# hritikbharucha/Custom_Porechop_ABI

Measured on AMD Instinct MI355X. Metric: reads/sec trimmed (100k ONT reads x 50 adapter pairs), higher is better.
Workload: dtype int32

## Files before the change

### custom_porechop_abi_amd/csrc/pcabi_dp.h

```cpp
#pragma once

#ifndef PCABI_ROW_FENCE
#define PCABI_ROW_FENCE 1
#endif
#ifndef PCABI_TAB_PD
#define PCABI_TAB_PD 0
#endif
#ifndef PCABI_TAB_PD_LONG
#define PCABI_TAB_PD_LONG 1
#endif

#include <stdint.h>
#include <algorithm>

#ifdef __HIPCC__
#define PCABI_HD __host__ __device__ __forceinline__
#else
#define PCABI_HD inline
#endif

namespace pcabi {

constexpr int NEG = -(1 << 28);

// ... 423 lines not shown
            best.b.bj = j;
            const int vt = LAST ? vt_up : 0, vp = LAST ? vp_up : 0;
            if (AFFINE) {
                if (lv == ls)      { best.c = lvc; best.n = lvn; best.b.ltype = LT_V; best.b.trail = vt; best.b.precd = vp; }
                else if (lh == ls) { best.c = lhc; best.n = lhn; best.b.ltype = LT_H; best.b.trail = ht; best.b.precd = hp; }
                else               { best.c = lsc; best.n = lsn; best.b.ltype = LT_D; best.b.trail = 0; best.b.precd = 0; }
            } else {
                best.c = lsc; best.n = lsn; best.b.ltype = lt_type;
                best.b.trail = (lt_type == LT_V) ? vt : (lt_type == LT_H ? ht : 0);
                best.b.precd = (lt_type == LT_V) ? vp : (lt_type == LT_H ? hp : 0);
            }
        }
        if (AFFINE || lt_type == LT_H) { ht_last = ht; hp_last = hp; }
        else { ht_last = 0; hp_last = 0; }
        slt_last = lt_type;
    }
};

template <int R, bool AFFINE, typename ReadFn, typename AdpFn, typename BndFn>
PCABI_HD Result align_lane_striped(const ReadFn &rd0, int n, AdpFn &adp, int L, int rt, const Scoring sc, BndFn &bnd,
                                   int own_lo = 1, int own_hi = -1) {
    const bool fin_read = own_hi < 0;
    const int hi = fin_read ? n + 1 : own_hi;
    const int pad = rt - L, k0 = pad / R, nst = rt / R;
    StripeDP<R, AFFINE> st;
    st.best.b.score = 0;
    st.best.b.bi = L;
    st.best.b.bj = 0;
    st.best.b.attr = 0;
    st.best.b.ltype = LT_NONE;
    st.best.b.trail = 0;
    st.best.b.precd = 0;
    st.best.c = -L;
    st.best.n = 0;
    st.bc = st.best;
    st.bc.b.score = SCORE_FLOOR;
    st.cslt = LT_NONE;
    st.cvt = 0;
    st.cvp = 0;
#pragma unroll 1
    for (int k = k0; k < nst; ++k) {
        adp.load(k);
        const bool first = k == k0, fin = k == nst - 1;
        const int off = first ? pad - k0 * R : 0;
        const int ib = k * R - pad;
        st.init_stripe(ib, off);
        ReadFn rd = rd0;
        BndCell up, nx, bot;
        auto row0 = [](int j, BndCell &u) { u.s = 0; u.v = NEG; u.sc = j; u.vc = 0; u.sn = 0; u.vn = 0; };
        if (first) row0(1, up);
        else bnd.load(1, up);
        int r = rd(1);
#pragma unroll 1
        for (int j = 1; j < n; ++j) {
            const int rn = rd(j + 1);
            if (first) row0(j + 1, nx);
            else bnd.load(j + 1, nx);
            st.template column<false>(r, j, up, adp, off, ib, L, fin, j >= own_lo && j < hi, sc, bot);
            if (!fin) bnd.store(j, bot);
            up = nx;
            r = rn;
        }
        if (fin_read) st.template column<true>(r, n, up, adp, off, ib, L, fin, n >= own_lo && n < hi, sc, bot);
        else st.template column<false>(r, n, up, adp, off, ib, L, fin, n >= own_lo && n < hi, sc, bot);
        if (!fin) bnd.store(n, bot);
    }
    return finish_path(st.best.b, st.best.c, (int)(st.best.n & 0xFFFFu), (int)(st.best.n >> 16), L,
                       fin_read ? n : n + 1);
}

}

namespace pcabi {

constexpr uint32_t INC_PAD = 1u << ATTR_CSH;

PCABI_HD int32_t vreg(int32_t x) {
#if defined(__HIP_DEVICE_COMPILE__)
    asm volatile("" : "+v"(x));
#endif
    return x;
}

PCABI_HD int max3i(int a, int b, int c) {
    const int ab = a > b ? a : b;
    return ab > c ? ab : c;
}
constexpr int PAD_CODE = 5;

template <int RPL, bool AFFINE>
struct LaneDP {
    int S[RPL + 1], H[RPL + 1];
    uint32_t SA[RPL + 1], HA[RPL + 1];
    int bscore, bi, bj, blt, btrail, bprec;
    uint32_t battr;
    int slt_last, ht_last, hp_last;
    int mis[4];
    uint32_t ids[4];

    template <typename AdpFn, bool LAST>
    PCABI_HD void column(const int r, const int j, const AdpFn &adp, const int L, const int off,
                         const Scoring &sc) {
        int sup = 0, vup = NEG;
        uint32_t saup = attr_start(j), vaup = 0;
        int slt_up = LT_NONE, vt_up = 0, vp_up = 0;
        int lv = 0, lh = 0, ls = 0, lslt = LT_D;
        bool lhext = false;
        uint32_t lva = 0, lha = 0, lsa = 0;
        bool match = (r == adp(1));
        int diag = 0 + (match ? sc.ma : mis[1]);
        uint32_t da = attr_start(j - 1) + ids[1] + (uint32_t)match;
#pragma unroll
        for (int s = 1; s <= RPL; ++s) {
            int diag_nx = 0;
            uint32_t da_nx = 0;
            if (s < RPL) {
                const bool mt = (r == adp(s + 1));
                const int mi_n = (s + 1 <= 3) ? mis[s + 1] : sc.mi;
                const uint32_t id_n = (s + 1 <= 3) ? ids[s + 1] : INC_D;
                diag_nx = S[s] + (mt ? sc.ma : mi_n);
                da_nx = SA[s] + id_n + (uint32_t)mt;
            }
            int hn, vn, sn;
            uint32_t han, van;
            bool hext, vext, fromv;
            if (AFFINE) {
                const int hx = H[s] + sc.ge, ho = S[s] + sc.go;
                hext = !(hx < ho);
                hn = hext ? hx : ho;
                han = hext ? HA[s] : SA[s];
                const int vx = vup + sc.ge, vo = sup + sc.go;
                vext = !(vx < vo);
                vn = vext ? vx : vo;
                van = vext ? vaup : saup;
            } else {
                hext = vext = false;
                vn = sup + sc.ge;
                hn = S[s] + sc.ge;
                van = saup;
                han = SA[s];
            }
            sn = max3i(diag, vn, hn);
            const bool isd = (diag == sn);
            fromv = (vn == sn);
            const uint32_t san = isd ? da : (fromv ? van : han);
            if (LAST && s < RPL) {
                const int slt = isd ? LT_D : (fromv ? LT_V : LT_H);
                const bool cont = AFFINE ? (vext || slt_up == LT_V) : (slt_up == LT_V);
                const int vt = cont ? vt_up + 1 : 1;
                const int vp = cont ? vp_up : (slt_up == LT_D ? 1 : 0);
                if (sn > bscore) {
                    bscore = sn;
                    bi = s - off;
                    bj = j;
                    if (AFFINE) {
                        const bool isv = (vn == sn), ish = !isv && (hn == sn);
                        battr = isv ? van : (ish ? han : san);
                        blt = isv ? LT_V : (ish ? LT_H : LT_D);
                        btrail = isv ? vt : 0;
                        bprec = isv ? vp : 0;
                    } else {
                        battr = san;
                        blt = slt;
                        btrail = (slt == LT_V) ? vt : 0;
                        bprec = (slt == LT_V) ? vp : 0;
                    }
// ... 632 lines not shown
    PCABI_HD void init(int L, const Scoring &sc, int P_, int B, int j0 = 0) {
        using pk::addw;
        const int off = RPL - L;
        P = P_;
        jj = j0;
        k_e = Y::sc(-sc.ge);
        k_eR = Y::sc(-sc.ge * RPL);
        k_rb = Y::sc(sc.ge * P);
        f0 = Y::sc(-B);
        kgo0 = Y::sc(sc.go - sc.ge) + ((P - 1) << Y::TB_SH);
        ftop = Y::sc(-sc.ge * j0 - B);
        kgo = kgo0 - j0 * Y::TAG1;
        int32_t fs = addw(ftop, kgo);
#pragma unroll
        for (int s = 1; s <= RPL; ++s) {
            fs = addw(fs, k_e);
            st.G[s] = addw(Y::start(off - s), fs);
            st.HK[s] = addw(fs, Y::sc(-1) + Y::TAG1);
        }
        st.bkey = Y::start(-L);
        st.bj = 0;
    }

    PCABI_HD void step() {
        ++jj;
        kgo -= Y::TAG1;
        ftop = pk::addw(ftop, k_e);
    }

    PCABI_HD void advance() {
        using pk::addw;
        step();
        if (jj == P) {
            const int32_t rb = addw(k_rb, P << Y::TB_SH);
#pragma unroll
            for (int s = 1; s <= RPL; ++s) {
                st.G[s] = addw(st.G[s], rb);
                st.HK[s] = addw(st.HK[s], rb);
            }
            jj = 0;
            kgo += P << Y::TB_SH;
            ftop = addw(ftop, k_rb);
        }
    }

    template <typename TabRow>
    PCABI_HD void column(const TabRow &tab, const int j, const int off) {
        using pk::addw;
        const int32_t kg = vreg(kgo);
        const int32_t top = addw(ftop, kgo);
        int32_t gup = addw(Y::start(j + off), top);
        int32_t vup = Y::SENT;
        int32_t diag = addw(addw(Y::start(j - 1 + off), top), Y::TAG1 - k_e);
        constexpr int NQ = RPL / 4;
        int32_t t[RPL + 2];
        if (PD > 0) {
#pragma unroll
            for (int q = 0; q <= PD && q < NQ; ++q) tab.quad(q, t + 4 * q + 1);
        }
        diag += (PD > 0 ? t[1] : tab(1));
        int32_t lv = 0, ls = 0;
#pragma unroll
        for (int s = 1; s <= RPL; ++s) {
            if (PD > 0 && (s & 3) == 1) {
                const int q = (s - 1) / 4 + PD + 1;
                if (q < NQ) tab.quad(q, t + 4 * q + 1);
            }
            int32_t diag_nx = 0;
            if (s < RPL) diag_nx = st.G[s] + (PD > 0 ? t[s + 1] : tab(s + 1));
            const int32_t hn = std::max(st.HK[s], st.G[s]);
            const int32_t vo = gup + Y::kv(s);
            const int32_t vn = std::max(vup, vo);
            const int32_t sn = max3i(diag, vn, hn);
            if (s == RPL) { lv = vn; ls = sn; }
            st.G[s] = (sn & ~Y::TAGM) + kg;
            st.HK[s] = hn;
            gup = st.G[s];
            vup = vn;
            diag = diag_nx;
#if defined(__HIP_DEVICE_COMPILE__)
            if (PCABI_ROW_FENCE > 0 && (s % (PCABI_ROW_FENCE > 0 ? PCABI_ROW_FENCE : 1)) == 0) __builtin_amdgcn_sched_barrier(0);
#endif
        }
        const int32_t corr = addw(std::max(lv, ls & ~Y::TAGM), pk::negw(addw(ftop, k_eR)));
        const bool upd = Y::score(corr) > Y::score(st.bkey);
        st.bkey = upd ? corr : st.bkey;
        st.bj = upd ? j : st.bj;
    }

    template <typename TabRow>
    PCABI_HD Result last_column(const TabRow &tab, const int n, const int L) {
        using pk::addw;
        using pk::negw;
        const int off = RPL - L;
        const int32_t ft = addw(f0, (int32_t)((uint32_t)jj * (uint32_t)k_e));
        const int32_t kgj = kgo0 - jj * Y::TAG1;
        const int32_t kg = vreg(kgj);
        const int32_t top = addw(ft, kgj);
        int32_t gup = addw(Y::start(n + off), top);
        int32_t vup = Y::SENT;
        int32_t diag = addw(addw(Y::start(n - 1 + off), top), Y::TAG1 - k_e);
        constexpr int NQ = RPL / 4;
        int32_t t[RPL + 2];
        if (PD > 0) {
#pragma unroll
            for (int q = 0; q <= PD && q < NQ; ++q) tab.quad(q, t + 4 * q + 1);
        }
        diag += (PD > 0 ? t[1] : tab(1));
        int32_t bkey = st.bkey;
        int brow = 0;
        int32_t un = negw(ft);
#pragma unroll
        for (int s = 1; s <= RPL; ++s) {
            if (PD > 0 && (s & 3) == 1) {
                const int q = (s - 1) / 4 + PD + 1;
                if (q < NQ) tab.quad(q, t + 4 * q + 1);
            }
            int32_t diag_nx = 0;
            if (s < RPL) diag_nx = st.G[s] + (PD > 0 ? t[s + 1] : tab(s + 1));
            const int32_t hn = std::max(st.HK[s], st.G[s]);
            const int32_t vo = gup + Y::kv(s);
            const int32_t vn = std::max(vup, vo);
            const int32_t sn = max3i(diag, vn, hn);
            const int32_t s0 = sn & ~Y::TAGM;
            un = addw(un, negw(k_e));
            const int32_t corr = addw(std::max(hn, s0), un);
            const bool upd = Y::score(corr) > Y::score(bkey);
            bkey = upd ? corr : bkey;
            brow = upd ? s : brow;
            gup = s0 + kg;
            vup = vn;
            diag = diag_nx;
#if defined(__HIP_DEVICE_COMPILE__)
            if (PCABI_ROW_FENCE > 0 && (s % (PCABI_ROW_FENCE > 0 ? PCABI_ROW_FENCE : 1)) == 0) __builtin_amdgcn_sched_barrier(0);
#endif
        }
        const bool last = brow != 0, tagged = Y::tb(bkey) != 0;
        Best b;
        b.score = Y::score(bkey);
        b.bi = last ? brow - off : L;
        b.bj = last ? n : st.bj;
        b.attr = Y::to_std(Y::attr(bkey), b.bj);
        b.ltype = last ? (tagged ? LT_H : LT_D) : (st.bj == 0 ? LT_NONE : (tagged ? LT_V : LT_D));
        b.trail = 0;
        b.precd = 0;
        return finish(b, L, n);
    }
};

template <int RPL, int PD = PCABI_TAB_PD, typename ReadFn, typename TabFn>
PCABI_HD Result align_lane_shift(ReadFn &rd, int n, const TabFn &tabfn, int L, const Scoring sc, int P, int B) {
    LaneShift<RPL, PD> ls;
    const int off = RPL - L;
    ls.init(L, sc, P, B);
    int r = rd(1);
#pragma unroll 1
    for (int j = 1; j < n; ++j) {
        const int rn = rd(j + 1);
        ls.advance();
        ls.template column<decltype(tabfn(r))>(tabfn(r), j, off);
        r = rn;
    }
    ls.advance();
    return ls.template last_column<decltype(tabfn(r))>(tabfn(r), n, L);
}

template <int RPL, int PD = PCABI_TAB_PD, typename TileFn, typename TabFn>
PCABI_HD Result align_lane_shift4(const TileFn &tr, int n, const TabFn &tabfn, int L, const Scoring sc, int P, int B) {
    LaneShift<RPL, PD> ls;
    const int off = RPL - L;
    ls.init(L, sc, P, B, -1);
    const int np = (n - 1) / 4;
    uint32_t cur = tr(0), nx = tr(1);
    int j = 1;
#pragma unroll 1
    for (int q = 0; q < np; ++q, j += 4) {
        const uint32_t w = cur;
        cur = nx;
        nx = tr(q + 2);
        ls.advance();
        ls.template column<decltype(tabfn(0))>(tabfn((int)(w & 0xFFu)), j, off);
        ls.step();
        ls.template column<decltype(tabfn(0))>(tabfn((int)((w >> 8) & 0xFFu)), j + 1, off);
        ls.step();
        ls.template column<decltype(tabfn(0))>(tabfn((int)((w >> 16) & 0xFFu)), j + 2, off);
        ls.step();
        ls.template column<decltype(tabfn(0))>(tabfn((int)(w >> 24)), j + 3, off);
    }
#pragma unroll 1
    for (; j < n; ++j) {
        ls.advance();
        ls.template column<decltype(tabfn(0))>(tabfn((int)((cur >> (8 * ((j - 1) & 3))) & 0xFFu)), j, off);
    }
    ls.advance();
    return ls.template last_column<decltype(tabfn(0))>(tabfn((int)((cur >> (8 * ((n - 1) & 3))) & 0xFFu)), n, L);
}

namespace pk {
template <int RPL, typename AdpFn>
PCABI_HD int32_t sub_key_pshift(int s, int c, const AdpFn &adp, int off, const Scoring &sc) {
    using Y = Lay<RPL>;
    const int d = -sc.go - sc.ge;
    if (s <= off) return Y::TB3 + Y::sc(d);
    return (c == adp(s)) ? (Y::sc(sc.ma + d) + Y::TB3 + Y::INC_M) : (Y::sc(sc.mi + d) + Y::TB3 + Y::INC_D);
}
constexpr int32_t PSENT = (int32_t)0x80000000;
}

template <int RPL, int PD = PCABI_TAB_PD>
struct LanePShift {
    using Y = pk::Lay<RPL>;
    LanePacked<RPL, true, Y, PD> st;
    int32_t kgo;
    int32_t ftop;
    int32_t f0;
    int32_t k_e;
    int32_t k_eR;
    int32_t k_rb;
    int jj, P;

    PCABI_HD void init(int L, const Scoring &sc, int P_, int B) {
        using pk::addw;
        const int off = RPL - L;
        P = P_;
        jj = 0;
        k_e = Y::sc(-sc.ge);
        k_eR = Y::sc(-sc.ge * RPL);
        k_rb = Y::sc(sc.ge * P);
        f0 = ftop = Y::sc(-B);
        kgo = Y::sc(sc.go - sc.ge);
        int32_t fs = vreg(addw(ftop, kgo));
#pragma unroll
        for (int s = 1; s <= RPL; ++s) {
            fs = addw(fs, k_e);
            st.G[s] = addw(Y::start(off - s), fs);
            st.HK[s] = addw(fs, Y::sc(-1)) | Y::TB1;
        }
        st.bkey = Y::start(-L);
        st.bj = 0;
    }

    PCABI_HD void advance() {
        using pk::addw;
        ++jj;
        ftop = addw(ftop, k_e);
        if (jj == P) {
#pragma unroll
            for (int s = 1; s <= RPL; ++s) {
                st.G[s] = addw(st.G[s], k_rb);
                st.HK[s] = addw(st.HK[s], k_rb);
            }
            jj = 0;
            ftop = addw(ftop, k_rb);
        }
    }

    template <typename TabRow>
    PCABI_HD void column(const TabRow &tab, const int j, const int off) {
        using pk::addw;
        const int32_t kg = vreg(kgo);
        const int32_t top = addw(ftop, kgo);
        int32_t gup = addw(Y::start(j + off), top);
        int32_t vup = pk::PSENT;
        int32_t diag = addw(addw(Y::start(j - 1 + off), top), pk::negw(k_e));
        constexpr int NQ = RPL / 4;
        int32_t t[RPL + 2];
        if (PD > 0) {
#pragma unroll
            for (int q = 0; q <= PD && q < NQ; ++q) tab.quad(q, t + 4 * q + 1);
        }
        diag = addw(diag, PD > 0 ? t[1] : tab(1));
        int32_t lv = 0, ls = 0;
#pragma unroll
        for (int s = 1; s <= RPL; ++s) {
            if (PD > 0 && (s & 3) == 1) {
// ... 472 lines not shown
```

### custom_porechop_abi_amd/csrc/pcabi_k_group.hip

```cpp
#include "pcabi_kern.h"

namespace pcabi_eng {

template <int CLS>
__global__ __launch_bounds__(256) void k_align_group(GroupParams gp) {
    constexpr int MAXR = group_max_rpl(CLS);
    __shared__ __attribute__((aligned(16))) int32_t tab[4 * kTabW * MAXR];
    int32_t *wave_tab = tab + (threadIdx.x >> 6) * kTabW * MAXR;
    const int64_t b = blockIdx.x;
    int s = 0;
    while (s + 1 < gp.n_seg && b >= gp.seg[s + 1].block0) ++s;
    const GroupSeg &g = gp.seg[s];
    KParams p{};
    p.tiles = g.tiles;
    p.tile_off = g.tile_off;
    p.win_len = g.win_len;
    p.n_win = g.n_win;
    p.adp_pad = g.adp_pad;
    p.adp_len = g.adp_len;
    p.adp_id = g.adp_id;
    p.n_adp = g.n_adp;
    p.out = g.out;
    p.out_stride = g.out_stride;
    p.sc = gp.sc;
    p.shift_p = g.shift_p;
    p.shift_b = g.shift_b;
    const int64_t lb = b - g.block0;
    if constexpr (CLS == 0) {
        if (g.shift_p > 0) {
            switch (g.rpl) {
#define T(R) case R: cross_block<R, true, SHIFT>(p, lb, wave_tab); break;
            T(4) T(8) T(12) T(16) T(20) T(24) T(28) T(32)
#undef T
            }
        } else {
            switch (g.rpl) {
#define T(R) case R: cross_block<R, true, TAGGED>(p, lb, wave_tab); break;
            T(4) T(8) T(12) T(16) T(20) T(24) T(28) T(32)
#undef T
            }
        }
    } else {
        if (g.shift_p > 0) {
            switch (g.rpl) {
#define P(R) case R: cross_block<R, true, PSHIFT>(p, lb, wave_tab); break;
            P(36) P(40) P(44) P(48) P(52) P(56) P(60) P(64)
#undef P
            }
        } else {
            switch (g.rpl) {
#define P(R) case R: cross_block<R, true, PACKED>(p, lb, wave_tab); break;
            P(36) P(40) P(44) P(48) P(52) P(56) P(60) P(64)
#undef P
            }
        }
    }
}

void dispatch_group(int cls, const GroupParams &p, int64_t blocks, hipStream_t st) {
    if (blocks <= 0) return;
    if (cls == 0) hipLaunchKernelGGL((k_align_group<0>), dim3((unsigned)blocks), dim3(256), 0, st, p);
    else hipLaunchKernelGGL((k_align_group<1>), dim3((unsigned)blocks), dim3(256), 0, st, p);
}

}
```

### custom_porechop_abi_amd/csrc/pcabi_kern.h

```cpp
#pragma once
#include <hip/hip_runtime.h>

#include <algorithm>
#include <cstdint>
#include <cstdlib>
#include <string>
#include <type_traits>

#include "../../include/pcabi.h"
#include "pcabi_dp.h"

#ifndef PCABI_WAVES
#define PCABI_WAVES 1
#endif

void pcabi_poison(void *p, size_t bytes);
void pcabi_poison_async(void *p, size_t bytes, hipStream_t st);

namespace pcabi_eng {

int fail(int code, const std::string &msg);

#define HIP_TRY(expr)                                                                   \
    do {                                                                                \
// ... 31 lines not shown
    const uint32_t *tiles;
    const int64_t *tile_off;
    const uint32_t *adp_pad;
    const int32_t *adp_len;
    const int32_t *adp_id;
    int32_t n_adp;
    const int32_t *task_win;
    const int32_t *task_out;
    const int32_t *wave_adp;
    int64_t n_waves;
    int32_t *out;
    int64_t out_stride;
    pcabi::Scoring sc;
    int32_t *compat;
    int32_t chunk_split;
    const int4 *task_chunk;
    int32_t rt;
    int32_t max_cols;
    int32_t *scratch;
    int64_t n_items;
    const int32_t *dev_waves;
    int32_t shift_p, shift_b;
};

struct WindowReader {
    const uint32_t *q;
    int64_t stride;
    int a8;
    uint32_t lo, hi, nx;
    __device__ __forceinline__ WindowReader() : q(nullptr), stride(0), a8(0), lo(0), hi(0), nx(0) {}
    __device__ __forceinline__ WindowReader(const uint32_t *base, int64_t stride_, int a8_)
        : q(base), stride(stride_), a8(a8_) {
        lo = q[0]; hi = q[stride]; nx = q[2 * stride];
    }
    __device__ __forceinline__ int operator()(int j) {
        const int k = j - 1;
        if (k > 0 && (k & 3) == 0) { lo = hi; hi = nx; nx = q[(int64_t)(k / 4 + 2) * stride]; }
        return (int)(((((uint64_t)hi << 32) | lo) >> (8 * (k & 3) + a8)) & 0xFFu);
    }
};

template <int RPL>
struct AdapterRegs {
    uint32_t w[RPL / 4];
    __device__ __forceinline__ void load(const uint32_t *src) {
#pragma unroll
        for (int k = 0; k < RPL / 4; ++k) w[k] = __builtin_amdgcn_readfirstlane(src[k]);
    }
    __device__ __forceinline__ int operator()(int s) const {
        return (int)((w[(s - 1) >> 2] >> (8 * ((s - 1) & 3))) & 0xFFu);
    }
};

__device__ __forceinline__ void store_result(int32_t *out, int64_t stride, int64_t idx,
                                             const pcabi::Result &r) {
    out[0 * stride + idx] = r.rs;
    out[1 * stride + idx] = r.re;
    out[2 * stride + idx] = r.as;
    out[3 * stride + idx] = r.ae;
    out[4 * stride + idx] = r.score;
    out[5 * stride + idx] = r.m;
    out[6 * stride + idx] = r.l1;
    out[7 * stride + idx] = r.l2;
}

__device__ __forceinline__ pcabi::Result empty_result() {
    pcabi::Result r;
    r.rs = -1; r.re = 0; r.as = -1; r.ae = 0;
    r.score = (int)0x80000000; r.m = 0; r.l1 = 0; r.l2 = 0;
    return r;
}

constexpr int kTabW = pcabi::pk::TAB_W;

struct LdsRow {
    const int32_t *p;
    __device__ __forceinline__ int32_t operator()(int s) const { return p[s - 1]; }
    __device__ __forceinline__ void quad(int q, int32_t *dst) const {
        const int4 v = *reinterpret_cast<const int4 *>(p + 4 * q);
        dst[0] = v.x; dst[1] = v.y; dst[2] = v.z; dst[3] = v.w;
    }
};

template <int RPL, typename Y = pcabi::pk::Lay<RPL>>
__device__ __forceinline__ void fill_wave_tab(const KParams &p, int a_local, int L, int32_t *wave_tab) {
    const int off = RPL - L;
    const int lane = threadIdx.x & 63;
    for (int e = lane; e < kTabW * RPL; e += 64) {
        const int c = e / RPL, srow = e % RPL + 1;
        const uint32_t *ap = p.adp_pad + (int64_t)a_local * (RPL / 4);
        auto code = [&](int sl) { return (int)((ap[(sl - 1) / 4] >> (8 * ((sl - 1) & 3))) & 0xFFu); };
        wave_tab[e] = pcabi::pk::sub_key<RPL, decltype(code), Y>(srow, c, code, off, p.sc);
    }
    __syncthreads();
}

template <int RPL>
__device__ __forceinline__ void fill_wave_tab_shift(const KParams &p, int a_local, int L, int32_t *wave_tab) {
    const int off = RPL - L;
    const int lane = threadIdx.x & 63;
    for (int e = lane; e < kTabW * RPL; e += 64) {
        const int c = e / RPL, srow = e % RPL + 1;
        const uint32_t *ap = p.adp_pad + (int64_t)a_local * (RPL / 4);
        auto code = [&](int sl) { return (int)((ap[(sl - 1) / 4] >> (8 * ((sl - 1) & 3))) & 0xFFu); };
        wave_tab[e] = pcabi::pk::sub_key_shift<RPL>(srow, c, code, off, p.sc);
    }
    __syncthreads();
}

template <int RPL>
__device__ __forceinline__ void fill_wave_tab_pshift(const KParams &p, int a_local, int L, int32_t *wave_tab) {
    const int off = RPL - L;
    const int lane = threadIdx.x & 63;
    for (int e = lane; e < kTabW * RPL; e += 64) {
        const int c = e / RPL, srow = e % RPL + 1;
        const uint32_t *ap = p.adp_pad + (int64_t)a_local * (RPL / 4);
        auto code = [&](int sl) { return (int)((ap[(sl - 1) / 4] >> (8 * ((sl - 1) & 3))) & 0xFFu); };
        wave_tab[e] = pcabi::pk::sub_key_pshift<RPL>(srow, c, code, off, p.sc);
    }
    __syncthreads();
}

template <int RPL>
__device__ __forceinline__ void fill_wave_tab_long(const KParams &p, int a_local, int L, int32_t *wave_tab) {
    const int off = RPL - L;
    const int lane = threadIdx.x & 63;
    const uint32_t *ap = p.adp_pad + (int64_t)a_local * (RPL / 4);
    auto code = [&](int sl) { return (int)((ap[(sl - 1) / 4] >> (8 * ((sl - 1) & 3))) & 0xFFu); };
    for (int e = lane; e < kTabW * RPL; e += 64) {
        const int c = e / RPL, srow = e % RPL + 1;
        wave_tab[e] = pcabi::pk::sub_key<RPL, decltype(code), pcabi::pk::LayL<RPL, 0>>(srow, c, code, off, p.sc);
        wave_tab[kTabW * RPL + e] =
            pcabi::pk::sub_key<RPL, decltype(code), pcabi::pk::LayL<RPL, 1>>(srow, c, code, off, p.sc);
    }
    __syncthreads();
}

constexpr int kShift4MaxRows = 24;

template <int RPL, bool AFFINE, int KIND>
__device__ __forceinline__ void run_lane(const KParams &p, int a_local, int64_t w, int64_t out_idx,
                                         int32_t *wave_tab, int64_t tile_off) {
    AdapterRegs<RPL> adp;
    if constexpr (KIND != LONG) adp.load(p.adp_pad + (int64_t)a_local * (RPL / 4));
    const int L = __builtin_amdgcn_readfirstlane(p.adp_len[a_local]);
    if constexpr (KIND == PACKED) fill_wave_tab<RPL>(p, a_local, L, wave_tab);
    if constexpr (KIND == TAGGED) fill_wave_tab<RPL, pcabi::pk::LayT<RPL>>(p, a_local, L, wave_tab);
    if constexpr (KIND == SHIFT) fill_wave_tab_shift<RPL>(p, a_local, L, wave_tab);
    if constexpr (KIND == PSHIFT) fill_wave_tab_pshift<RPL>(p, a_local, L, wave_tab);
    if constexpr (KIND == LONG) fill_wave_tab_long<RPL>(p, a_local, L, wave_tab);
    if (w < 0) return;
    const int n = p.win_len[w];
    pcabi::Result r;
    bool uniform = false;
    if constexpr (KIND == SHIFT) {
        const int n0 = __builtin_amdgcn_readfirstlane(n);
        const int P = __builtin_amdgcn_readfirstlane(p.shift_p);
        if (RPL <= kShift4MaxRows && n0 > 0 && (P & 3) == 0 && __builtin_amdgcn_ballot_w64(n != n0 || tile_off < 0) == 0) {
            const uint32_t *base = p.tiles + tile_off + (threadIdx.x & 255);
            auto tr = [&](int q) { return base[(int64_t)q * 256]; };
            auto tabfn = [&](int rc) { return LdsRow{wave_tab + rc * RPL}; };
            r = pcabi::align_lane_shift4<RPL>(tr, n0, tabfn, L, p.sc, P, p.shift_b);
            uniform = true;
        }
    }
    if (uniform) {
    } else if (n <= 0) {
        r = empty_result();
    } else {
        WindowReader rd = tile_off >= 0
            ? WindowReader(p.tiles + tile_off + (threadIdx.x & 255), 256, 0)
            : [&] {
                  const uint8_t *b = p.codes + p.win_off[w];
                  const int a0 = (int)((uintptr_t)b & 3);
                  return WindowReader(reinterpret_cast<const uint32_t *>(b - a0), 1, 8 * a0);
              }();
        if constexpr (KIND == PACKED) {
            auto tabfn = [&](int rc) { return LdsRow{wave_tab + rc * RPL}; };
            r = pcabi::align_lane_packed<(RPL <= pcabi::pk::MAX_RPL ? RPL : 4), AFFINE>(rd, n, tabfn, L, p.sc);
        } else if constexpr (KIND == TAGGED) {
            static_assert(RPL <= 32 && AFFINE, "run-tagged layout: affine buckets of <= 32 rows");
            auto tabfn = [&](int rc) { return LdsRow{wave_tab + rc * RPL}; };
            r = pcabi::align_lane_packed<RPL, true, false, pcabi::pk::LayT<RPL>>(rd, n, tabfn, L, p.sc);
        } else if constexpr (KIND == SHIFT) {
            static_assert(RPL <= 32 && AFFINE, "gap-extend frame: affine buckets of <= 32 rows");
            auto tabfn = [&](int rc) { return LdsRow{wave_tab + rc * RPL}; };
            r = pcabi::align_lane_shift<RPL>(rd, n, tabfn, L, p.sc, p.shift_p, p.shift_b);
        } else if constexpr (KIND == PSHIFT) {
            static_assert(RPL >= 36 && RPL <= 64 && AFFINE, "packed gap-extend frame: affine buckets of 36..64 rows");
            auto tabfn = [&](int rc) { return LdsRow{wave_tab + rc * RPL}; };
            r = pcabi::align_lane_pshift<RPL>(rd, n, tabfn, L, p.sc, p.shift_p, p.shift_b);
        } else if constexpr (KIND == LONG) {
            WindowReader rd1 = rd;
            auto tab0 = [&](int rc) { return LdsRow{wave_tab + rc * RPL}; };
            auto tab1 = [&](int rc) { return LdsRow{wave_tab + kTabW * RPL + rc * RPL}; };
            r = pcabi::align_lane_packed_long<RPL, AFFINE>(rd, rd1, n, tab0, tab1, L, p.sc);
        } else if constexpr (KIND == FAST) {
            r = pcabi::align_lane_fast<RPL, AFFINE>(rd, n, adp, L, p.sc);
        } else {
            r = pcabi::align_lane_generic<RPL, AFFINE>(rd, n, adp, L, p.sc);
        }
    }
    if (p.compat) {
        int en_match = 0;
        if (r.rs >= 0 && r.diag_en && r.l1 > 0) {
            const uint8_t *ab = reinterpret_cast<const uint8_t *>(p.adp_pad + (int64_t)a_local * (RPL / 4));
            en_match = p.codes[p.win_off[w] + r.re] == ab[RPL - L + r.ae];
        }
        p.compat[out_idx] = pcabi::compat_flag(r, n, en_match);
        return;
    }
    store_result(p.out, p.out_stride, out_idx, r);
}

template <int KIND, int RPL>
constexpr int wave_tab_ints() {
    return (KIND == PACKED || KIND == TAGGED || KIND == SHIFT || KIND == PSHIFT) ? kTabW * RPL : (KIND == LONG ? 2 * kTabW * RPL : 1);
}

template <int RPL, bool AFFINE, int KIND>
__device__ __forceinline__ void cross_block(const KParams &p, int64_t b, int32_t *wave_tab) {
    const int64_t k = b >> 3;
    const int a_local = (int)(k % p.n_adp);
    const int64_t tile = (k / p.n_adp) * 8 + (b & 7);
    const int64_t w = tile * 256 + threadIdx.x;
    const int a_glob = p.adp_id[a_local];
    const int64_t toff = w < p.n_win ? p.tile_off[tile] : 0;
    run_lane<RPL, AFFINE, KIND>(p, a_local, w < p.n_win ? w : -1, (int64_t)a_glob * p.n_win + w, wave_tab, toff);
}

template <int RPL, bool AFFINE, int KIND>
__global__ __launch_bounds__(256, PCABI_WAVES) void k_align(KParams p) {
    __shared__ __attribute__((aligned(16))) int32_t tab[4 * wave_tab_ints<KIND, RPL>()];
    int32_t *wave_tab = tab + (threadIdx.x >> 6) * wave_tab_ints<KIND, RPL>();
    if (p.task_win == nullptr) {
        cross_block<RPL, AFFINE, KIND>(p, blockIdx.x, wave_tab);
    } else {
        int64_t wave = (int64_t)blockIdx.x * 4 + (threadIdx.x >> 6);
        const bool live = wave < p.n_waves;
        if (!live) wave = p.n_waves - 1;
        const int64_t slot = wave * 64 + (threadIdx.x & 63);
        const int a_local = __builtin_amdgcn_readfirstlane(p.wave_adp[wave]);
        const int32_t tw = live ? p.task_win[slot] : -1;
        run_lane<RPL, AFFINE, KIND>(p, a_local, tw, tw >= 0 ? p.task_out[slot] : 0, wave_tab, -1);
    }
}

struct FParams {
    const uint32_t *tiles;
    const int64_t *tile_off;
    const int32_t *win_len;
    int64_t n_win;
    const uint32_t *adp_pad;
    const int32_t *adp_len;
    const int32_t *adp_id;
    int32_t n_adp;
    int16_t *s16;
    pcabi::Scoring sc;
};

struct LdsRow16 {
    const int32_t *p;
    __device__ __forceinline__ void quad(int q, pcabi::sf::v2 *dst) const {
        const int4 v = *reinterpret_cast<const int4 *>(p + 4 * q);
        dst[0] = __builtin_bit_cast(pcabi::sf::v2, v.x);
        dst[1] = __builtin_bit_cast(pcabi::sf::v2, v.y);
        dst[2] = __builtin_bit_cast(pcabi::sf::v2, v.z);
        dst[3] = __builtin_bit_cast(pcabi::sf::v2, v.w);
    }
};

template <int RPL, bool AFFINE>
__global__ __launch_bounds__(256) void k_score_filter(FParams p) {
    __shared__ __attribute__((aligned(16))) int32_t tab[4 * kTabW * RPL];
    int32_t *wave_tab = tab + (threadIdx.x >> 6) * kTabW * RPL;
    const int n_pair = (p.n_adp + 1) / 2;
    const int64_t b = blockIdx.x;
    const int64_t k = b >> 3;
    const int pr = (int)(k % n_pair);
    const int64_t tile = (k / n_pair) * 8 + (b & 7);
    const int64_t w = tile * 256 + threadIdx.x;
    const int ia = 2 * pr, ib = (2 * pr + 1 < p.n_adp) ? 2 * pr + 1 : 2 * pr;
    const int La = __builtin_amdgcn_readfirstlane(p.adp_len[ia]);
    const int Lb = __builtin_amdgcn_readfirstlane(p.adp_len[ib]);
    {
        const int lane = threadIdx.x & 63;
        const uint32_t *pa = p.adp_pad + (int64_t)ia * (RPL / 4), *pb = p.adp_pad + (int64_t)ib * (RPL / 4);
        for (int e = lane; e < kTabW * RPL; e += 64) {
            const int c = e / RPL, sl = e % RPL + 1;
            const int ca = (int)((pa[(sl - 1) / 4] >> (8 * ((sl - 1) & 3))) & 0xFFu);
            const int cb = (int)((pb[(sl - 1) / 4] >> (8 * ((sl - 1) & 3))) & 0xFFu);
            const int va = sl <= RPL - La ? 0 : (c == ca ? p.sc.ma : p.sc.mi);
            const int vb = sl <= RPL - Lb ? 0 : (c == cb ? p.sc.ma : p.sc.mi);
            const uint32_t lo = (uint16_t)(int16_t)(va - p.sc.go), hi = (uint16_t)(int16_t)(vb - p.sc.go);
            wave_tab[e] = (int32_t)(lo | (hi << 16));
        }
        __syncthreads();
    }
    if (w >= p.n_win) return;
    const int n = p.win_len[w];
    WindowReader rd(p.tiles + p.tile_off[tile] + threadIdx.x, 256, 0);
    auto tabfn = [&](int rc) { return LdsRow16{wave_tab + rc * RPL}; };
    const pcabi::sf::v2 r = pcabi::filter_lane<RPL, AFFINE>(rd, n, tabfn, p.sc);
    p.s16[(int64_t)p.adp_id[ia] * p.n_win + w] = r[0];
    if (ib != ia) p.s16[(int64_t)p.adp_id[ib] * p.n_win + w] = r[1];
}

template <int RPL, bool AFFINE, int KIND>
__device__ __forceinline__ void chunk_wave(const KParams &p, int64_t wave, bool live, int32_t *wave_tab) {
    const int64_t slot = wave * 64 + (threadIdx.x & 63);
    const int a_local = __builtin_amdgcn_readfirstlane(p.wave_adp[wave]);
    const int L = __builtin_amdgcn_readfirstlane(p.adp_len[a_local]);
    if constexpr (KIND == PACKED) fill_wave_tab<RPL>(p, a_local, L, wave_tab);
    if constexpr (KIND == TAGGED) fill_wave_tab<RPL, pcabi::pk::LayT<RPL>>(p, a_local, L, wave_tab);
    if constexpr (KIND == LONG) fill_wave_tab_long<RPL>(p, a_local, L, wave_tab);
    const int32_t tw = live ? p.task_win[slot] : -1;
    if (tw < 0) return;
    const int4 ck = p.task_chunk[slot];
    const uint8_t *b = p.codes + p.win_off[tw] + ck.x;
    const int a0 = (int)((uintptr_t)b & 3);
// ... 361 lines not shown
```

Before: 17.44 million.

## Share block-wide score table, branch-skip best update, unroll shift4 by eight

In cross_block launches, all four waves of a block work on the same adapter, so the substitution table is now built once per block by all 256 threads into a single shared array. This replaces four per-wave copies, cutting LDS footprint and fill work. The per-column best-score update in the shift kernel now computes a cheap upper-bound test and skips the max/select work when no lane improves, using a wave ballot. The uniform shift4 column loop now processes eight columns per iteration with reordered tile prefetch. The tail loop swaps in the next word every four columns.

```diff
diff --git a/custom_porechop_abi_amd/csrc/pcabi_dp.h b/custom_porechop_abi_amd/csrc/pcabi_dp.h
--- a/custom_porechop_abi_amd/csrc/pcabi_dp.h
+++ b/custom_porechop_abi_amd/csrc/pcabi_dp.h
@@ -529,6 +529,17 @@
     return x;
 }
 
+#ifndef PCABI_SCOUT_BRANCH
+#define PCABI_SCOUT_BRANCH 1
+#endif
+PCABI_HD bool any_lane(bool b) {
+#if defined(__HIP_DEVICE_COMPILE__)
+    return PCABI_SCOUT_BRANCH == 0 || __builtin_amdgcn_ballot_w64(b) != 0;
+#else
+    return b;
+#endif
+}
+
 PCABI_HD int max3i(int a, int b, int c) {
     const int ab = a > b ? a : b;
     return ab > c ? ab : c;
@@ -1327,10 +1338,13 @@
             if (PCABI_ROW_FENCE > 0 && (s % (PCABI_ROW_FENCE > 0 ? PCABI_ROW_FENCE : 1)) == 0) __builtin_amdgcn_sched_barrier(0);
 #endif
         }
-        const int32_t corr = addw(std::max(lv, ls & ~Y::TAGM), pk::negw(addw(ftop, k_eR)));
-        const bool upd = Y::score(corr) > Y::score(st.bkey);
-        st.bkey = upd ? corr : st.bkey;
-        st.bj = upd ? j : st.bj;
+        const int32_t un = pk::negw(addw(ftop, k_eR));
+        const bool upd = Y::score(addw(ls, un)) > Y::score(st.bkey);
+        if (any_lane(upd)) {
+            const int32_t corr = vreg(addw(std::max(lv, ls & ~Y::TAGM), un));
+            st.bkey = upd ? corr : st.bkey;
+            st.bj = upd ? j : st.bj;
+        }
     }
 
     template <typename TabRow>
@@ -1415,14 +1429,7 @@
     LaneShift<RPL, PD> ls;
     const int off = RPL - L;
     ls.init(L, sc, P, B, -1);
-    const int np = (n - 1) / 4;
-    uint32_t cur = tr(0), nx = tr(1);
-    int j = 1;
-#pragma unroll 1
-    for (int q = 0; q < np; ++q, j += 4) {
-        const uint32_t w = cur;
-        cur = nx;
-        nx = tr(q + 2);
+    auto pass = [&](const uint32_t w, const int j) {
         ls.advance();
         ls.template column<decltype(tabfn(0))>(tabfn((int)(w & 0xFFu)), j, off);
         ls.step();
@@ -1431,11 +1438,23 @@
         ls.template column<decltype(tabfn(0))>(tabfn((int)((w >> 16) & 0xFFu)), j + 2, off);
         ls.step();
         ls.template column<decltype(tabfn(0))>(tabfn((int)(w >> 24)), j + 3, off);
-    }
+    };
+    const int np2 = (n - 1) / 8;
+    uint32_t cur = tr(0);
+    int j = 1;
+#pragma unroll 1
+    for (int q = 0; q < np2; ++q, j += 8) {
+        const uint32_t nx = tr(2 * q + 1);
+        pass(cur, j);
+        cur = tr(2 * q + 2);
+        pass(nx, j + 4);
+    }
+    const uint32_t nx = tr(2 * np2 + 1);
 #pragma unroll 1
     for (; j < n; ++j) {
         ls.advance();
         ls.template column<decltype(tabfn(0))>(tabfn((int)((cur >> (8 * ((j - 1) & 3))) & 0xFFu)), j, off);
+        if ((j & 3) == 0) cur = nx;
     }
     ls.advance();
     return ls.template last_column<decltype(tabfn(0))>(tabfn((int)((cur >> (8 * ((n - 1) & 3))) & 0xFFu)), n, L);
diff --git a/custom_porechop_abi_amd/csrc/pcabi_k_group.hip b/custom_porechop_abi_amd/csrc/pcabi_k_group.hip
--- a/custom_porechop_abi_amd/csrc/pcabi_k_group.hip
+++ b/custom_porechop_abi_amd/csrc/pcabi_k_group.hip
@@ -5,8 +5,7 @@
 template <int CLS>
 __global__ __launch_bounds__(256) void k_align_group(GroupParams gp) {
     constexpr int MAXR = group_max_rpl(CLS);
-    __shared__ __attribute__((aligned(16))) int32_t tab[4 * kTabW * MAXR];
-    int32_t *wave_tab = tab + (threadIdx.x >> 6) * kTabW * MAXR;
+    __shared__ __attribute__((aligned(16))) int32_t tab[kTabW * MAXR];
     const int64_t b = blockIdx.x;
     int s = 0;
     while (s + 1 < gp.n_seg && b >= gp.seg[s + 1].block0) ++s;
@@ -29,13 +28,13 @@
     if constexpr (CLS == 0) {
         if (g.shift_p > 0) {
             switch (g.rpl) {
-#define T(R) case R: cross_block<R, true, SHIFT>(p, lb, wave_tab); break;
+#define T(R) case R: cross_block<R, true, SHIFT>(p, lb, tab); break;
             T(4) T(8) T(12) T(16) T(20) T(24) T(28) T(32)
 #undef T
             }
         } else {
             switch (g.rpl) {
-#define T(R) case R: cross_block<R, true, TAGGED>(p, lb, wave_tab); break;
+#define T(R) case R: cross_block<R, true, TAGGED>(p, lb, tab); break;
             T(4) T(8) T(12) T(16) T(20) T(24) T(28) T(32)
 #undef T
             }
@@ -43,13 +42,13 @@
     } else {
         if (g.shift_p > 0) {
             switch (g.rpl) {
-#define P(R) case R: cross_block<R, true, PSHIFT>(p, lb, wave_tab); break;
+#define P(R) case R: cross_block<R, true, PSHIFT>(p, lb, tab); break;
             P(36) P(40) P(44) P(48) P(52) P(56) P(60) P(64)
 #undef P
             }
         } else {
             switch (g.rpl) {
-#define P(R) case R: cross_block<R, true, PACKED>(p, lb, wave_tab); break;
+#define P(R) case R: cross_block<R, true, PACKED>(p, lb, tab); break;
             P(36) P(40) P(44) P(48) P(52) P(56) P(60) P(64)
 #undef P
             }
diff --git a/custom_porechop_abi_amd/csrc/pcabi_kern.h b/custom_porechop_abi_amd/csrc/pcabi_kern.h
--- a/custom_porechop_abi_amd/csrc/pcabi_kern.h
+++ b/custom_porechop_abi_amd/csrc/pcabi_kern.h
@@ -137,73 +137,58 @@
     }
 };
 
-template <int RPL, typename Y = pcabi::pk::Lay<RPL>>
-__device__ __forceinline__ void fill_wave_tab(const KParams &p, int a_local, int L, int32_t *wave_tab) {
-    const int off = RPL - L;
-    const int lane = threadIdx.x & 63;
-    for (int e = lane; e < kTabW * RPL; e += 64) {
-        const int c = e / RPL, srow = e % RPL + 1;
-        const uint32_t *ap = p.adp_pad + (int64_t)a_local * (RPL / 4);
-        auto code = [&](int sl) { return (int)((ap[(sl - 1) / 4] >> (8 * ((sl - 1) & 3))) & 0xFFu); };
-        wave_tab[e] = pcabi::pk::sub_key<RPL, decltype(code), Y>(srow, c, code, off, p.sc);
-    }
-    __syncthreads();
-}
-
-template <int RPL>
-__device__ __forceinline__ void fill_wave_tab_shift(const KParams &p, int a_local, int L, int32_t *wave_tab) {
-    const int off = RPL - L;
-    const int lane = threadIdx.x & 63;
-    for (int e = lane; e < kTabW * RPL; e += 64) {
-        const int c = e / RPL, srow = e % RPL + 1;
-        const uint32_t *ap = p.adp_pad + (int64_t)a_local * (RPL / 4);
-        auto code = [&](int sl) { return (int)((ap[(sl - 1) / 4] >> (8 * ((sl - 1) & 3))) & 0xFFu); };
-        wave_tab[e] = pcabi::pk::sub_key_shift<RPL>(srow, c, code, off, p.sc);
-    }
-    __syncthreads();
-}
-
-template <int RPL>
-__device__ __forceinline__ void fill_wave_tab_pshift(const KParams &p, int a_local, int L, int32_t *wave_tab) {
-    const int off = RPL - L;
-    const int lane = threadIdx.x & 63;
-    for (int e = lane; e < kTabW * RPL; e += 64) {
-        const int c = e / RPL, srow = e % RPL + 1;
-        const uint32_t *ap = p.adp_pad + (int64_t)a_local * (RPL / 4);
-        auto code = [&](int sl) { return (int)((ap[(sl - 1) / 4] >> (8 * ((sl - 1) & 3))) & 0xFFu); };
-        wave_tab[e] = pcabi::pk::sub_key_pshift<RPL>(srow, c, code, off, p.sc);
-    }
-    __syncthreads();
-}
-
-template <int RPL>
-__device__ __forceinline__ void fill_wave_tab_long(const KParams &p, int a_local, int L, int32_t *wave_tab) {
-    const int off = RPL - L;
-    const int lane = threadIdx.x & 63;
+template <int RPL, bool BLOCK, typename PutFn>
+__device__ __forceinline__ void fill_tab(const KParams &p, int a_local, const PutFn &put) {
     const uint32_t *ap = p.adp_pad + (int64_t)a_local * (RPL / 4);
     auto code = [&](int sl) { return (int)((ap[(sl - 1) / 4] >> (8 * ((sl - 1) & 3))) & 0xFFu); };
-    for (int e = lane; e < kTabW * RPL; e += 64) {
-        const int c = e / RPL, srow = e % RPL + 1;
-        wave_tab[e] = pcabi::pk::sub_key<RPL, decltype(code), pcabi::pk::LayL<RPL, 0>>(srow, c, code, off, p.sc);
-        wave_tab[kTabW * RPL + e] =
-            pcabi::pk::sub_key<RPL, decltype(code), pcabi::pk::LayL<RPL, 1>>(srow, c, code, off, p.sc);
-    }
+    for (int e = BLOCK ? (int)threadIdx.x : (int)(threadIdx.x & 63); e < kTabW * RPL; e += BLOCK ? 256 : 64)
+        put(e, e % RPL + 1, e / RPL, code);
     __syncthreads();
 }
 
+template <int RPL, typename Y = pcabi::pk::Lay<RPL>, bool BLOCK = false>
+__device__ __forceinline__ void fill_wave_tab(const KParams &p, int a_local, int L, int32_t *tab) {
+    fill_tab<RPL, BLOCK>(p, a_local, [&](int e, int srow, int c, const auto &code) {
+        tab[e] = pcabi::pk::sub_key<RPL, decltype(code), Y>(srow, c, code, RPL - L, p.sc);
+    });
+}
+
+template <int RPL, bool BLOCK = false>
+__device__ __forceinline__ void fill_wave_tab_shift(const KParams &p, int a_local, int L, int32_t *tab) {
+    fill_tab<RPL, BLOCK>(p, a_local, [&](int e, int srow, int c, const auto &code) {
+        tab[e] = pcabi::pk::sub_key_shift<RPL>(srow, c, code, RPL - L, p.sc);
+    });
+}
+
+template <int RPL, bool BLOCK = false>
+__device__ __forceinline__ void fill_wave_tab_pshift(const KParams &p, int a_local, int L, int32_t *tab) {
+    fill_tab<RPL, BLOCK>(p, a_local, [&](int e, int srow, int c, const auto &code) {
+        tab[e] = pcabi::pk::sub_key_pshift<RPL>(srow, c, code, RPL - L, p.sc);
+    });
+}
+
+template <int RPL, bool BLOCK = false>
+__device__ __forceinline__ void fill_wave_tab_long(const KParams &p, int a_local, int L, int32_t *tab) {
+    fill_tab<RPL, BLOCK>(p, a_local, [&](int e, int srow, int c, const auto &code) {
+        tab[e] = pcabi::pk::sub_key<RPL, decltype(code), pcabi::pk::LayL<RPL, 0>>(srow, c, code, RPL - L, p.sc);
+        tab[kTabW * RPL + e] =
+            pcabi::pk::sub_key<RPL, decltype(code), pcabi::pk::LayL<RPL, 1>>(srow, c, code, RPL - L, p.sc);
+    });
+}
+
 constexpr int kShift4MaxRows = 24;
 
-template <int RPL, bool AFFINE, int KIND>
+template <int RPL, bool AFFINE, int KIND, bool BLOCK = false>
 __device__ __forceinline__ void run_lane(const KParams &p, int a_local, int64_t w, int64_t out_idx,
                                          int32_t *wave_tab, int64_t tile_off) {
     AdapterRegs<RPL> adp;
     if constexpr (KIND != LONG) adp.load(p.adp_pad + (int64_t)a_local * (RPL / 4));
     const int L = __builtin_amdgcn_readfirstlane(p.adp_len[a_local]);
-    if constexpr (KIND == PACKED) fill_wave_tab<RPL>(p, a_local, L, wave_tab);
-    if constexpr (KIND == TAGGED) fill_wave_tab<RPL, pcabi::pk::LayT<RPL>>(p, a_local, L, wave_tab);
-    if constexpr (KIND == SHIFT) fill_wave_tab_shift<RPL>(p, a_local, L, wave_tab);
-    if constexpr (KIND == PSHIFT) fill_wave_tab_pshift<RPL>(p, a_local, L, wave_tab);
-    if constexpr (KIND == LONG) fill_wave_tab_long<RPL>(p, a_local, L, wave_tab);
+    if constexpr (KIND == PACKED) fill_wave_tab<RPL, pcabi::pk::Lay<RPL>, BLOCK>(p, a_local, L, wave_tab);
+    if constexpr (KIND == TAGGED) fill_wave_tab<RPL, pcabi::pk::LayT<RPL>, BLOCK>(p, a_local, L, wave_tab);
+    if constexpr (KIND == SHIFT) fill_wave_tab_shift<RPL, BLOCK>(p, a_local, L, wave_tab);
+    if constexpr (KIND == PSHIFT) fill_wave_tab_pshift<RPL, BLOCK>(p, a_local, L, wave_tab);
+    if constexpr (KIND == LONG) fill_wave_tab_long<RPL, BLOCK>(p, a_local, L, wave_tab);
     if (w < 0) return;
     const int n = p.win_len[w];
     pcabi::Result r;
@@ -274,23 +259,23 @@
 }
 
 template <int RPL, bool AFFINE, int KIND>
-__device__ __forceinline__ void cross_block(const KParams &p, int64_t b, int32_t *wave_tab) {
+__device__ __forceinline__ void cross_block(const KParams &p, int64_t b, int32_t *tab) {
     const int64_t k = b >> 3;
     const int a_local = (int)(k % p.n_adp);
     const int64_t tile = (k / p.n_adp) * 8 + (b & 7);
     const int64_t w = tile * 256 + threadIdx.x;
     const int a_glob = p.adp_id[a_local];
     const int64_t toff = w < p.n_win ? p.tile_off[tile] : 0;
-    run_lane<RPL, AFFINE, KIND>(p, a_local, w < p.n_win ? w : -1, (int64_t)a_glob * p.n_win + w, wave_tab, toff);
+    run_lane<RPL, AFFINE, KIND, true>(p, a_local, w < p.n_win ? w : -1, (int64_t)a_glob * p.n_win + w, tab, toff);
 }
 
 template <int RPL, bool AFFINE, int KIND>
 __global__ __launch_bounds__(256, PCABI_WAVES) void k_align(KParams p) {
     __shared__ __attribute__((aligned(16))) int32_t tab[4 * wave_tab_ints<KIND, RPL>()];
-    int32_t *wave_tab = tab + (threadIdx.x >> 6) * wave_tab_ints<KIND, RPL>();
     if (p.task_win == nullptr) {
-        cross_block<RPL, AFFINE, KIND>(p, blockIdx.x, wave_tab);
+        cross_block<RPL, AFFINE, KIND>(p, blockIdx.x, tab);
     } else {
+        int32_t *wave_tab = tab + (threadIdx.x >> 6) * wave_tab_ints<KIND, RPL>();
         int64_t wave = (int64_t)blockIdx.x * 4 + (threadIdx.x >> 6);
         const bool live = wave < p.n_waves;
         if (!live) wave = p.n_waves - 1;
```

After: 17.42 million. Within noise of the previous version (-0.1%).
